# parsakhaz/multimodal-image-similarity-search

Measured on AMD Instinct MI355X. Metric: images/s CLIP-B/32 encode @ bs256; Mvec/s cosine top-10 over 10M x 512, higher is better.
Workload: dtype bf16

## Files before the change

multimodal-image-similarity-search_amd/csrc/api_index.hip:

```cpp
#include "common.h"
#include <queue>
#include "retrieval_kernels.h"
#include "gemm_bf16_256.h"
#include "gemm_bf16_p256.h"
#include <algorithm>

struct mmiss_index {
    int dim = 0, dtype = MMISS_F32, device = 0, elt = 4;
    int qelt() const { return dtype == MMISS_F32 ? 4 : 2; }
    hipStream_t own_stream = nullptr, user_stream = nullptr;
    bool has_user_stream = false;
    hipEvent_t done_ev = nullptr;
    bool async_pending = false;
    std::mutex mu;
    int64_t count = 0, capacity = 0;
    DevBuf rows, labels_d;
    DevBuf inv;
    std::vector<int64_t> labels_h;
    DevBuf tags;
    std::vector<uint64_t> tags_h;
    DevBuf fmask, fmask2, tag_stage;
    DevBuf stage, qn, qs, qstage, lists_s, lists_r, lists2_s, lists2_r, cand, cur_s, cur_r, out_c, map, gmax;
    DevBuf qmap, qmap64, qs2, cand2;
    DevBuf eps_q, thr, thr2, swp_cnt, swp_list;
    DevBuf seed_s, seed_r, fcnt, fbuf_s, fbuf_g;
    PinBuf pin;
    PinBuf swp_pin;
    int64_t stat_queries = 0, stat_flagged = 0, stat_rounds = 0, stat_pages = 0, stat_exhaustive = 0, stat_swept_rows = 0;
    struct Pending {
        bool active = false, out_dev = false, guard = false;
        int Q = 0, k = 0;
        int64_t* d_lab = nullptr; float* d_dist = nullptr; int32_t* d_cnt = nullptr; int32_t* h_flags = nullptr;
        int64_t* out_labels = nullptr; float* out_dist = nullptr; int32_t* out_count = nullptr;
        bool filt = false;
        std::vector<uint64_t> req, exc;
        const uint64_t* d_mask = nullptr;
    } pend;
    DevBuf dist_all;
    PinBuf dist_pin;
    hipStream_t stream() const { return has_user_stream ? user_stream : own_stream; }
};

#define MM_NO_PENDING(ix, who) \
    do { if ((ix)->pend.active) MM_FAIL(MMISS_ERR_STATE, "%s: a query begun with mmiss_index_query_begin is still open", who); } while (0)

namespace {

template <typename T_, typename Q_, typename Bits_> struct Storage { using T = T_; using Q = Q_; using Bits = Bits_; };
template <typename F> auto with_storage(int dtype, F&& f) {
    if (dtype == MMISS_F16) return f(Storage<_Float16, _Float16, _Float16>{});
    if (dtype == MMISS_F8) return f(Storage<F8, _Float16, uint8_t>{});
    return f(Storage<float, float, float>{});
}
template <typename S> constexpr bool is_f8 = std::is_same<typename S::T, F8>::value;

struct RowStore {
    DevBuf rows, labels, inv, tags;
    int alloc(const mmiss_index* ix, int64_t cap, hipStream_t st) {
        MM_TRY(rows.alloc((size_t)cap * ix->dim * ix->elt));
        MM_TRY(labels.alloc((size_t)cap * 8));
        MM_TRY(tags.alloc((size_t)cap * 8));
        MM_HIP(hipMemsetAsync(tags.p, 0, (size_t)cap * 8, st));
        if (ix->dtype == MMISS_F8) {
            MM_TRY(inv.alloc((size_t)cap * 4));
            MM_HIP(hipMemsetAsync(inv.p, 0, (size_t)cap * 4, st));
        }
        return MMISS_OK;
    }
};

void swap_rows(mmiss_index* ix, RowStore& s) { ix->rows.swap(s.rows); ix->labels_d.swap(s.labels); ix->inv.swap(s.inv); ix->tags.swap(s.tags); }

int reset_rows(mmiss_index* ix, hipStream_t st) {
    ix->count = 0;
    ix->labels_h.clear();
    ix->tags_h.clear();
    if (ix->capacity == 0) return MMISS_OK;
    if (ix->dtype == MMISS_F8) MM_HIP(hipMemsetAsync(ix->inv.p, 0, (size_t)ix->capacity * 4, st));
    MM_HIP(hipMemsetAsync(ix->tags.p, 0, (size_t)ix->capacity * 8, st));
    MM_HIP(hipStreamSynchronize(st));
    return MMISS_OK;
}

// ... 174 lines not shown
    if (!out) MM_FAIL(MMISS_ERR_ARG, "mmiss_index_create: null out");
    if (dim <= 0 || dim % 128 || dim > 4096) MM_FAIL(MMISS_ERR_UNSUPPORTED, "index dim %d: need a multiple of 128, <= 4096", dim);
    if (storage_dtype != MMISS_F32 && storage_dtype != MMISS_F16 && storage_dtype != MMISS_F8)
        MM_FAIL(MMISS_ERR_ARG, "unknown storage dtype %d", storage_dtype);
    if (scan_lds_bytes(dim, storage_dtype == MMISS_F32 ? 4 : 2, 1, 64) > SCAN_LDS_LIMIT)
        MM_FAIL(MMISS_ERR_UNSUPPORTED, "index dim %d with storage dtype %d: a 16-query block of the scan needs %d bytes of LDS (limit %d); "
                "f32 rows go up to dim 1920, f16 / fp8 rows up to 3968", dim, storage_dtype,
                scan_lds_bytes(dim, storage_dtype == MMISS_F32 ? 4 : 2, 1, 64), SCAN_LDS_LIMIT);
    MM_TRY(mmiss_use_device(device));
    mmiss_index* ix = new (std::nothrow) mmiss_index();
    if (!ix) MM_FAIL(MMISS_ERR_NOMEM, "out of host memory");
    ix->dim = dim; ix->dtype = storage_dtype; ix->device = device; ix->elt = storage_dtype == MMISS_F16 ? 2 : storage_dtype == MMISS_F8 ? 1 : 4;
    if (hipStreamCreateWithFlags(&ix->own_stream, hipStreamNonBlocking) != hipSuccess) {
        delete ix;
        MM_FAIL(MMISS_ERR_HIP, "hipStreamCreate failed");
    }
    if (hipEventCreateWithFlags(&ix->done_ev, hipEventDisableTiming) != hipSuccess) {
        (void)hipStreamDestroy(ix->own_stream);
        delete ix;
        MM_FAIL(MMISS_ERR_HIP, "hipEventCreate failed");
    }
    if (capacity_hint > 0) {
        int rc = index_reserve(ix, capacity_hint, ix->own_stream);
        if (rc != MMISS_OK) {
            (void)hipStreamDestroy(ix->own_stream); (void)hipEventDestroy(ix->done_ev);
            delete ix;
            return rc;
        }
    }
    *out = ix;
    return MMISS_OK;
}

extern "C" int mmiss_index_destroy(mmiss_index* ix) {
    if (!ix) return MMISS_OK;
    (void)hipSetDevice(ix->device);
    (void)hipDeviceSynchronize();
    if (ix->own_stream) (void)hipStreamDestroy(ix->own_stream);
    if (ix->done_ev) (void)hipEventDestroy(ix->done_ev);
    delete ix;
    return MMISS_OK;
}

extern "C" int mmiss_index_set_stream(mmiss_index* ix, void* hip_stream, int32_t use_own) {
    if (!ix) MM_FAIL(MMISS_ERR_ARG, "null index");
    std::lock_guard<std::mutex> lk(ix->mu);
    MM_NO_PENDING(ix, "mmiss_index_set_stream");
    hipStream_t next = reinterpret_cast<hipStream_t>(hip_stream);
    const bool next_user = use_own == 0;
    if (next_user != ix->has_user_stream || (next_user && next != ix->user_stream)) {
        MM_TRY(mmiss_use_device(ix->device));
        if (ix->async_pending) MM_HIP(hipEventSynchronize(ix->done_ev));
        ix->async_pending = false;
    }
    ix->user_stream = next;
    ix->has_user_stream = next_user;
    return MMISS_OK;
}

extern "C" int mmiss_index_count(mmiss_index* ix, int64_t* count) {
    if (!ix || !count) MM_FAIL(MMISS_ERR_ARG, "mmiss_index_count: null argument");
    std::lock_guard<std::mutex> lk(ix->mu);
    *count = ix->count;
    return MMISS_OK;
}

extern "C" int mmiss_index_clear(mmiss_index* ix) {
    if (!ix) MM_FAIL(MMISS_ERR_ARG, "null index");
    std::lock_guard<std::mutex> lk(ix->mu);
    MM_NO_PENDING(ix, "mmiss_index_clear");
    if (ix->capacity > 0) MM_TRY(mmiss_use_device(ix->device));
    return reset_rows(ix, ix->stream());
}

extern "C" int mmiss_index_add(mmiss_index* ix, const float* vecs, const int64_t* labels, int64_t n) {
    if (!ix || (n > 0 && (!vecs || !labels))) MM_FAIL(MMISS_ERR_ARG, "mmiss_index_add: null argument");
    if (n < 0) MM_FAIL(MMISS_ERR_ARG, "mmiss_index_add: n = %lld", (long long)n);
    if (n == 0) return MMISS_OK;
    std::lock_guard<std::mutex> lk(ix->mu);
    MM_NO_PENDING(ix, "mmiss_index_add");
    MM_TRY(mmiss_use_device(ix->device));
    hipStream_t st = ix->stream();
    std::vector<int64_t> lab;
    MM_TRY(fetch_i64(labels, n, lab));
    int64_t prev = ix->labels_h.empty() ? INT64_MIN : ix->labels_h.back();
    for (int64_t i = 0; i < n; ++i) {
        if (lab[i] < 0) MM_FAIL(MMISS_ERR_ARG, "mmiss_index_add: negative label %lld", (long long)lab[i]);
        if (lab[i] <= prev)
            MM_FAIL(MMISS_ERR_ARG, "mmiss_index_add: labels must be strictly increasing (label %lld after %lld)",
                    (long long)lab[i], (long long)prev);
        prev = lab[i];
    }
    if (ix->count + n >= (int64_t)INT32_MAX - 64) MM_FAIL(MMISS_ERR_UNSUPPORTED, "index shard limited to 2^31 rows");
    MM_TRY(index_reserve(ix, ix->count + n, st));
    const int D = ix->dim;
    const bool in_dev = mmiss_is_device_ptr(vecs);
    const int64_t chunk = 1 << 16;
    for (int64_t r0 = 0; r0 < n; r0 += chunk) {
        const int64_t nr = std::min(chunk, n - r0);
        const float* src = vecs + r0 * D;
        if (!in_dev) {
            MM_TRY(ix->stage.ensure((size_t)chunk * D * 4));
            MM_HIP(hipMemcpyAsync(ix->stage.p, src, (size_t)nr * D * 4, hipMemcpyHostToDevice, st));
            src = ix->stage.as<float>();
        }
        MM_TRY(launch_normalize(ix, src, ix->rows.as<char>() + (size_t)(ix->count + r0) * D * ix->elt, nr, st, ix->count + r0));
        if (!in_dev) MM_HIP(hipStreamSynchronize(st));
    }
    MM_HIP(hipMemcpyAsync(ix->labels_d.as<int64_t>() + ix->count, lab.data(), (size_t)n * 8, hipMemcpyHostToDevice, st));
    MM_HIP(hipStreamSynchronize(st));
    ix->labels_h.insert(ix->labels_h.end(), lab.begin(), lab.end());
    ix->tags_h.resize((size_t)(ix->count + n), 0);
    ix->count += n;
    return MMISS_OK;
}

extern "C" int mmiss_index_update(mmiss_index* ix, const int64_t* labels, const float* vecs, int64_t n) {
    if (!ix || (n > 0 && (!vecs || !labels))) MM_FAIL(MMISS_ERR_ARG, "mmiss_index_update: null argument");
    if (n <= 0) return n == 0 ? MMISS_OK : MMISS_ERR_ARG;
    std::lock_guard<std::mutex> lk(ix->mu);
    MM_NO_PENDING(ix, "mmiss_index_update");
    MM_TRY(mmiss_use_device(ix->device));
    hipStream_t st = ix->stream();
    std::vector<int64_t> lab;
    MM_TRY(fetch_i64(labels, n, lab));
    std::vector<int64_t> rows((size_t)n);
    for (int64_t i = 0; i < n; ++i) {
        rows[i] = find_row(ix, lab[i]);
        if (rows[i] < 0) MM_FAIL(MMISS_ERR_ARG, "mmiss_index_update: label %lld not in the index", (long long)lab[i]);
    }
    const int D = ix->dim;
    const float* src = vecs;
    if (!mmiss_is_device_ptr(vecs)) {
        MM_TRY(ix->stage.ensure((size_t)n * D * 4));
        MM_HIP(hipMemcpyAsync(ix->stage.p, vecs, (size_t)n * D * 4, hipMemcpyHostToDevice, st));
        src = ix->stage.as<float>();
    }
    for (int64_t i = 0; i < n; ++i)
        MM_TRY(launch_normalize(ix, src + i * D, ix->rows.as<char>() + (size_t)rows[i] * D * ix->elt, 1, st, rows[i]));
    MM_HIP(hipStreamSynchronize(st));
    return MMISS_OK;
}

extern "C" int mmiss_index_remove(mmiss_index* ix, const int64_t* labels, int64_t n, int64_t* removed) {
    if (!ix || (n > 0 && !labels)) MM_FAIL(MMISS_ERR_ARG, "mmiss_index_remove: null argument");
    if (removed) *removed = 0;
    if (n <= 0) return n == 0 ? MMISS_OK : MMISS_ERR_ARG;
    std::lock_guard<std::mutex> lk(ix->mu);
    MM_NO_PENDING(ix, "mmiss_index_remove");
    MM_TRY(mmiss_use_device(ix->device));
    hipStream_t st = ix->stream();
    std::vector<int64_t> lab;
    MM_TRY(fetch_i64(labels, n, lab));
    std::vector<char> drop((size_t)ix->count, 0);
    int64_t ndrop = 0;
    for (int64_t i = 0; i < n; ++i) {
        const int64_t r = find_row(ix, lab[i]);
        if (r >= 0 && !drop[r]) { drop[r] = 1; ++ndrop; }
    }
    if (removed) *removed = ndrop;
    if (ndrop == 0) return MMISS_OK;
    const int64_t keep = ix->count - ndrop;
    if (keep == 0) return reset_rows(ix, st);
    std::vector<int64_t> map((size_t)keep), nl((size_t)keep);
    std::vector<uint64_t> ntag((size_t)keep);
    for (int64_t r = 0, o = 0; r < ix->count; ++r)
        if (!drop[r]) { map[o] = r; nl[o] = ix->labels_h[r]; ntag[o] = ix->tags_h[r]; ++o; }
    RowStore fresh;
    MM_TRY(fresh.alloc(ix, ix->capacity, st));
    MM_HIP(hipMemcpyAsync(fresh.tags.p, ntag.data(), (size_t)keep * 8, hipMemcpyHostToDevice, st));
    MM_TRY(ix->map.ensure((size_t)keep * 8));
    MM_HIP(hipMemcpyAsync(ix->map.p, map.data(), (size_t)keep * 8, hipMemcpyHostToDevice, st));
    with_storage(ix->dtype, [&](auto s) {
        using B = typename decltype(s)::Bits;
        hipLaunchKernelGGL(gather_rows_kernel<B>, dim3((int)std::min<int64_t>(4096, (keep * ix->dim + 255) / 256)), dim3(256), 0, st,
                           ix->rows.as<B>(), ix->map.as<int64_t>(), fresh.rows.as<B>(), keep, ix->dim);
        if constexpr (is_f8<decltype(s)>)
            hipLaunchKernelGGL(gather_rows_kernel<float>, dim3((int)std::min<int64_t>(4096, (keep + 255) / 256)), dim3(256), 0, st,
                               ix->inv.as<float>(), ix->map.as<int64_t>(), fresh.inv.as<float>(), keep, 1);
    });
    MM_HIP(hipGetLastError());
    MM_HIP(hipMemcpyAsync(fresh.labels.p, nl.data(), (size_t)keep * 8, hipMemcpyHostToDevice, st));
    MM_HIP(hipStreamSynchronize(st));
    swap_rows(ix, fresh);
    ix->labels_h.swap(nl);
    ix->tags_h.swap(ntag);
    ix->count = keep;
    return MMISS_OK;
}

extern "C" int mmiss_index_get(mmiss_index* ix, const int64_t* labels, int64_t n, float* out) {
    if (!ix || (n > 0 && (!labels || !out))) MM_FAIL(MMISS_ERR_ARG, "mmiss_index_get: null argument");
    if (n <= 0) return n == 0 ? MMISS_OK : MMISS_ERR_ARG;
    std::lock_guard<std::mutex> lk(ix->mu);
    MM_NO_PENDING(ix, "mmiss_index_get");
    MM_TRY(mmiss_use_device(ix->device));
    hipStream_t st = ix->stream();
    std::vector<int64_t> lab;
    MM_TRY(fetch_i64(labels, n, lab));
    std::vector<int64_t> map((size_t)n);
    for (int64_t i = 0; i < n; ++i) {
        map[i] = find_row(ix, lab[i]);
// ... 146 lines not shown
            else if (Ent(d, (int32_t)r) < heap.top()) { heap.pop(); heap.push(Ent(d, (int32_t)r)); }
        }
        int32_t* c = cand.data() + (size_t)i * kkpad;
        for (size_t j = 0; !heap.empty(); ++j) { c[j] = heap.top().second; heap.pop(); }
        ix->stat_exhaustive += 1;
    }
    MM_TRY(ix->cand2.ensure((size_t)nq * kkpad * 4));
    MM_TRY(ix->qmap.ensure((size_t)nq * 4));
    MM_HIP(hipMemcpyAsync(ix->cand2.p, cand.data(), (size_t)nq * kkpad * 4, hipMemcpyHostToDevice, st));
    MM_HIP(hipMemcpyAsync(ix->qmap.p, which.data(), (size_t)nq * 4, hipMemcpyHostToDevice, st));
    RerankArgs r{};
    r.rows = ix->rows.p; r.D = D; r.inv = ix->inv.as<float>(); r.qn = ix->qn.as<float>(); r.cand = ix->cand2.as<int32_t>();
    r.cand_stride = kkpad; r.ncand = kkpad; r.group_mode = 0; r.nrows = N;
    r.labels = ix->labels_d.as<int64_t>(); r.k = pd.k;
    r.out_labels = pd.d_lab; r.out_dist = pd.d_dist; r.out_count = pd.d_cnt;
    r.qmap = ix->qmap.as<int32_t>();
    MM_TRY(launch_rerank(ix, st, r, nq));
    MM_HIP(hipStreamSynchronize(st));
    return MMISS_OK;
}

int strip_length(int Mq, int64_t nbn, int64_t ncol) {
    const int64_t tiles = nbn * (Mq / 256);
    int strip = (int)std::min<int64_t>(32, std::max<int64_t>(1, tiles / 2048));
    if (strip >= 8 && mmiss_option("score_strip_fit", 1) != 0) {
        double best = 1e300;
        int best_s = strip;
        for (int sl = strip; sl >= strip / 2; --sl) {
            const int64_t wgs = (Mq / 256) * ((ncol + sl - 1) / sl);
            const int64_t rounds = (wgs + 255) / 256;
            const double cost = (double)rounds * (sl + 0.25);
            if (cost < best - 1e-9) { best = cost; best_s = sl; }
        }
        strip = best_s;
    }
    const int forced = mmiss_option("score_strip", 0);
    if (forced > 0) strip = forced;
    return strip;
}

bool strip_v3(const mmiss_index* ix) { return mmiss_option("score_strip_v3", 1) != 0 && (ix->dim % 128) == 0 && ix->dim >= 256; }

bool strip_gemm_rows(const mmiss_index* ix) {
    return ix->dtype == MMISS_F16 || (ix->dtype == MMISS_F8 && mmiss_option("score_f8_gemm", 1) != 0);
}

int launch_strip_gemm(mmiss_index* ix, hipStream_t st, bool v3, const void* qs, const GemmEpi& ep, int M, int N, int strip,
                      const StripFilter* flt) {
    if (ix->dtype == MMISS_F8) return launch_gemm256s<_Float16, true>(st, qs, ix->rows.p, ep, M, N, ix->dim, strip, flt);
    if (v3) return launch_gemm256s<_Float16>(st, qs, ix->rows.p, ep, M, N, ix->dim, strip, flt);
    return launch_gemm256_strip<_Float16>(st, qs, ix->rows.p, ep, M, N, ix->dim, strip, flt);
}

int sweep_queries(mmiss_index* ix, hipStream_t st, const mmiss_index::Pending& pd, const std::vector<int32_t>& which) {
    const int Qf = (int)which.size(), D = ix->dim;
    const int64_t N = ix->count;
    if (Qf == 0 || N <= 0) return MMISS_OK;
    const bool gemm = !pd.filt && strip_gemm_rows(ix) && strip_v3(ix) && Qf > mmiss_option("sweep_gemm_min_q", 64);
    const int Qfp = (int)round_up(Qf, 256);
    MM_TRY(ix->swp_cnt.ensure((size_t)Qfp * 4));
    MM_TRY(ix->swp_list.ensure((size_t)Qf * SWEEP_CAP * 4));
    MM_HIP(hipMemsetAsync(ix->swp_cnt.p, 0, (size_t)Qfp * 4, st));
    const bool all = Qf == pd.Q;
    const void* qs_sw = ix->qs.p;
    const float* thr_sw = ix->thr.as<float>();
    const int32_t* qmap_sw = nullptr;
    const uint64_t* fm_sw = pd.d_mask;
    std::vector<uint64_t> fm2;
    if (!all && pd.filt) {
        fm2.resize((size_t)Qf * 2);
        for (int i = 0; i < Qf; ++i) { fm2[i] = pd.req[(size_t)which[i]]; fm2[Qf + i] = pd.exc[(size_t)which[i]]; }
        MM_TRY(ix->fmask2.ensure((size_t)Qf * 16));
        MM_HIP(hipMemcpyAsync(ix->fmask2.p, fm2.data(), (size_t)Qf * 16, hipMemcpyHostToDevice, st));
        fm_sw = ix->fmask2.as<uint64_t>();
    }
    if (!all) {
        std::vector<int64_t> map64(which.begin(), which.end());
        MM_TRY(ix->qmap.ensure((size_t)Qf * 4));
        MM_TRY(ix->qmap64.ensure((size_t)Qf * 8));
        MM_TRY(ix->qs2.ensure((size_t)Qfp * D * ix->qelt()));
        MM_TRY(ix->thr2.ensure((size_t)Qfp * 4));
        MM_HIP(hipMemcpyAsync(ix->qmap.p, which.data(), (size_t)Qf * 4, hipMemcpyHostToDevice, st));
        MM_HIP(hipMemcpyAsync(ix->qmap64.p, map64.data(), (size_t)Qf * 8, hipMemcpyHostToDevice, st));
        MM_HIP(hipStreamSynchronize(st));
        if (Qfp > Qf) MM_HIP(hipMemsetAsync(ix->qs2.as<char>() + (size_t)Qf * D * ix->qelt(), 0, (size_t)(Qfp - Qf) * D * ix->qelt(), st));
        with_storage(ix->dtype, [&](auto s) {
            using QT = typename decltype(s)::Q;
            hipLaunchKernelGGL(gather_rows_kernel<QT>, dim3((int)std::min<int64_t>(4096, ((int64_t)Qf * D + 255) / 256)), dim3(256), 0, st,
                               ix->qs.as<QT>(), ix->qmap64.as<int64_t>(), ix->qs2.as<QT>(), (int64_t)Qf, D);
        });
        MM_HIP(hipGetLastError());
        hipLaunchKernelGGL(gather_rows_kernel<float>, dim3((Qf + 255) / 256), dim3(256), 0, st, ix->thr.as<float>(),
                           ix->qmap64.as<int64_t>(), ix->thr2.as<float>(), (int64_t)Qf, 1);
        MM_HIP(hipGetLastError());
        qs_sw = ix->qs2.p; thr_sw = ix->thr2.as<float>(); qmap_sw = ix->qmap.as<int32_t>();
    }
    if (gemm) {
        const int64_t Npad = round_up(N, 256), nbn = Npad / 256;
        GemmEpi ep{};
        ep.m_valid = Qf; ep.p0 = (int)N; ep.m_fast = 1;
        ep.aux = ix->inv.as<float>();
        StripFilter flt{};
        flt.tau = thr_sw; flt.tau_stride = 1; flt.cnt = ix->swp_cnt.as<int32_t>();
        flt.buf_s = nullptr; flt.buf_g = ix->swp_list.as<int32_t>(); flt.cap = SWEEP_CAP; flt.bn_begin = 0;
        const int strip = strip_length(Qfp, nbn, nbn);
        MM_PROF(ix->dtype == MMISS_F8 ? "sweep_gemm_f8" : "sweep_gemm_f16", st, 2.0 * Qf * (double)N * D, (double)N * D * ix->elt);
        MM_TRY(launch_strip_gemm(ix, st, true, qs_sw, ep, Qfp, (int)Npad, strip, &flt));
        ix->stat_pages += 1;
    } else {
        const ScanPlan p = plan_sweep(D, ix->qelt(), Qf, N);
        if (p.lds > SCAN_LDS_LIMIT)
            MM_FAIL(MMISS_ERR_UNSUPPORTED, "widen pass: a 16-query block of dim %d does not fit the LDS (%d bytes)", D, p.lds);
        ScanArgs a{};
        a.rows = ix->rows.p; a.N = N; a.D = D; a.inv = ix->inv.as<float>(); a.qs = qs_sw; a.Q = Qf;
        a.thr = thr_sw; a.gcnt = ix->swp_cnt.as<int32_t>(); a.glist = ix->swp_list.as<int32_t>(); a.gcap = SWEEP_CAP;
        if (pd.filt) { a.tags = ix->tags.as<uint64_t>(); a.req = fm_sw; a.exc = fm_sw + Qf; }
        a.tiles_per_block = p.tiles_per_block;
        MM_TRY(launch_scan(ix, st, a, p));
        ix->stat_pages += p.qtiles;
    }
    const int SWEEP_FAST = 1024;
    RerankArgs r{};
    r.rows = ix->rows.p; r.D = D; r.inv = ix->inv.as<float>(); r.qn = ix->qn.as<float>(); r.cand = ix->swp_list.as<int32_t>();
    r.cand_stride = SWEEP_CAP; r.ncand = SWEEP_FAST; r.cand_cnt = ix->swp_cnt.as<int32_t>();
    r.group_mode = 0; r.nrows = N;
    r.labels = ix->labels_d.as<int64_t>(); r.k = pd.k;
    r.out_labels = pd.d_lab; r.out_dist = pd.d_dist; r.out_count = pd.d_cnt;
    r.qmap = qmap_sw;
    MM_TRY(ix->swp_pin.ensure((size_t)Qf * 4, st, (size_t)(Qf < 1024 ? 1024 : 2 * Qf) * 4));
    r.cnt_host = ix->swp_pin.as<int32_t>();
    MM_TRY(launch_rerank(ix, st, r, Qf));
    r.cnt_host = nullptr;
    MM_HIP(hipStreamSynchronize(st));
    const int32_t* cnt = ix->swp_pin.as<int32_t>();
    ix->stat_rounds += 1;
    std::vector<int32_t> big_b, rest;
    int maxc = 1;
    for (int b = 0; b < Qf; ++b) {
        if (cnt[b] > SWEEP_CAP) rest.push_back(which[b]);
        else {
            ix->stat_swept_rows += cnt[b];
            if (cnt[b] > SWEEP_FAST) { big_b.push_back(b); maxc = std::max(maxc, cnt[b]); }
        }
    }
    if (!big_b.empty()) {
        const int nb = (int)big_b.size();
        std::vector<int32_t> qm((size_t)nb);
        for (int j = 0; j < nb; ++j) qm[j] = which[big_b[j]];
        MM_TRY(ix->cand2.ensure((size_t)nb * 8));
        MM_HIP(hipMemcpyAsync(ix->cand2.p, big_b.data(), (size_t)nb * 4, hipMemcpyHostToDevice, st));
        MM_HIP(hipMemcpyAsync(ix->cand2.as<int32_t>() + nb, qm.data(), (size_t)nb * 4, hipMemcpyHostToDevice, st));
        MM_HIP(hipStreamSynchronize(st));
        r.ncand = (int)round_up(maxc, 32);
        r.bmap = ix->cand2.as<int32_t>();
        r.qmap = ix->cand2.as<int32_t>() + nb;
        MM_TRY(launch_rerank(ix, st, r, nb));
    }
    MM_TRY(exhaustive_queries(ix, st, pd, rest));
    MM_HIP(hipStreamSynchronize(st));
    return MMISS_OK;
}

}

namespace {

struct QueryPlan {
    int kp = 0, pages = 0, ncand = 0;
    bool dense = false;
    bool dense8 = false;
    bool big = false;
    bool strip_v3 = false;
    bool sample = false;
    int Mq = 0, strip = 1, filter_cap = 0;
    int64_t Npad = 0, nbn = 0, ns_tiles = 0, Ndense = 0;
};

int plan_query(const mmiss_index* ix, int Q, int k, bool filt, QueryPlan& p) {
    const int64_t N = ix->count;
    const int64_t want = std::min<int64_t>(k, N);
    if (want <= 10) { p.kp = 16; p.pages = 1; }
    else if (want <= 24) { p.kp = 32; p.pages = 1; }
    else {
        p.kp = 32;
        p.pages = (int)((std::min<int64_t>(want + 8, N) + 31) / 32);
    }
    p.ncand = p.kp * p.pages;
    if (p.ncand > 2048) MM_FAIL(MMISS_ERR_UNSUPPORTED, "mmiss_index_query: k = %d too large (max 2040)", k);

    const bool single = !filt && N > 0 && p.pages == 1;
    p.big = Q >= mmiss_option("score_big_min_q", 129);
    p.strip_v3 = strip_v3(ix);
    p.dense8 = single && ix->dtype == MMISS_F8 && p.big && p.strip_v3 && strip_gemm_rows(ix);
    p.dense = (single && ix->dtype == MMISS_F16 && Q > 16) || p.dense8;
    if (!p.dense) return MMISS_OK;
    p.Npad = round_up(N, p.big ? 256 : 128);
    p.Mq = (int)round_up(Q, p.big ? 256 : 128);
    p.nbn = p.Npad / 256;
    p.ns_tiles = std::max<int64_t>(16, p.nbn / std::max(1, mmiss_option("score_sample_div", 32)));
    const int filter_opt = mmiss_option("score_filter", 1);
    p.sample = p.big && p.nbn >= 128 && filter_opt != 0 && (filter_opt == 2 || (double)p.Mq * (double)p.Npad >= 1e9);
    p.Ndense = p.sample ? p.ns_tiles * 256 : p.Npad;
    if (p.big) p.strip = strip_length(p.Mq, p.nbn, p.sample ? p.nbn - p.ns_tiles : p.nbn);
    if (p.sample) p.filter_cap = mmiss_option("score_filter_cap", 2048);
    return MMISS_OK;
}

int stage_filter(mmiss_index* ix, hipStream_t st, int Q, const uint64_t* req, const uint64_t* exc) {
    mmiss_index::Pending& pd = ix->pend;
    pd.filt = req || exc;
    pd.d_mask = nullptr;
    if (!pd.filt) return MMISS_OK;
    if (req) MM_TRY(fetch_u64(req, Q, pd.req, st)); else pd.req.assign((size_t)Q, 0);
// ... 129 lines not shown
        MM_HIP(hipMemcpyAsync(ix->cur_s.p, inf.data(), (size_t)Q * 4, hipMemcpyHostToDevice, st));
        MM_HIP(hipMemcpyAsync(ix->cur_r.p, neg.data(), (size_t)Q * 4, hipMemcpyHostToDevice, st));
        MM_HIP(hipStreamSynchronize(st));
    }
    for (int page = 0; page < qp.pages; ++page) {
        ScanArgs a{};
        a.rows = ix->rows.p; a.N = ix->count; a.D = ix->dim; a.inv = ix->inv.as<float>(); a.qs = ix->qs.p; a.Q = Q;
        a.cur_s = paging ? ix->cur_s.as<float>() : nullptr;
        a.cur_r = paging ? ix->cur_r.as<int32_t>() : nullptr;
        a.kp = kp; a.tiles_per_block = p.tiles_per_block;
        a.out_s = ix->lists_s.as<float>(); a.out_r = ix->lists_r.as<int32_t>();
        if (pd.filt) { a.tags = ix->tags.as<uint64_t>(); a.req = pd.d_mask; a.exc = pd.d_mask + Q; }
        MM_TRY(launch_scan(ix, st, a, p));
        MergeArgs m{};
        m.in_s = ix->lists_s.as<float>(); m.in_r = ix->lists_r.as<int32_t>();
        m.L = p.slabs; m.Q = Q; m.kp = kp;
        m.cand = ix->cand.as<int32_t>(); m.cand_stride = qp.ncand; m.page_off = page * kp;
        m.cur_s = ix->cur_s.as<float>(); m.cur_r = ix->cur_r.as<int32_t>();
        MM_TRY(launch_merge(ix, st, m));
    }
    return MMISS_OK;
}

int rerank_first(mmiss_index* ix, hipStream_t st, const QueryPlan& p) {
    const mmiss_index::Pending& pd = ix->pend;
    RerankArgs r{};
    r.rows = ix->rows.p; r.D = ix->dim; r.inv = ix->inv.as<float>(); r.qn = ix->qn.as<float>(); r.cand = ix->cand.as<int32_t>();
    r.cand_stride = p.ncand; r.ncand = p.dense ? p.ncand * 16 : p.ncand; r.group_mode = p.dense ? 1 : 0; r.nrows = ix->count;
    r.labels = ix->labels_d.as<int64_t>(); r.k = pd.k;
    r.out_labels = pd.d_lab; r.out_dist = pd.d_dist; r.out_count = pd.d_cnt;
    if (pd.guard) {
        r.tau = ix->cur_s.as<float>(); r.eps_q = ix->eps_q.as<float>();
        r.thr_out = ix->thr.as<float>();
        r.flags = pd.h_flags; r.nflag = nullptr;
        r.force_flag = mmiss_option("guard_force", 0);
        if (p.sample) { r.ovf_cnt = ix->fcnt.as<int32_t>(); r.ovf_cap = p.filter_cap; }
    }
    return launch_rerank(ix, st, r, pd.Q);
}

int query_begin_locked(mmiss_index* ix, const float* queries, int32_t Q, int32_t k, const uint64_t* req, const uint64_t* exc,
                       int64_t* out_labels, float* out_dist, int32_t* out_count) {
    MM_TRY(mmiss_use_device(ix->device));
    hipStream_t st = ix->stream();
    const int64_t N = ix->count;
    mmiss_index::Pending& pd = ix->pend;
    pd.out_dev = mmiss_is_device_ptr(out_labels);
    if (pd.out_dev != mmiss_is_device_ptr(out_dist) || (out_count && pd.out_dev != mmiss_is_device_ptr(out_count)))
        MM_FAIL(MMISS_ERR_ARG, "mmiss_index_query: output pointers must be all host or all device");
    MM_TRY(stage_filter(ix, st, Q, req, exc));
    MM_TRY(stage_outputs(ix, st, Q, k, out_labels, out_dist, out_count));
    QueryPlan p;
    MM_TRY(plan_query(ix, Q, k, pd.filt, p));
    MM_TRY(upload_queries(ix, st, queries, Q));
    MM_TRY(ix->cand.ensure((size_t)Q * p.ncand * 4));
    MM_TRY(ix->cur_s.ensure((size_t)Q * 4));
    MM_TRY(ix->cur_r.ensure((size_t)Q * 4));
    if (N == 0) MM_HIP(hipMemsetAsync(ix->cand.p, 0xff, (size_t)Q * p.ncand * 4, st));
    else if (p.dense) MM_TRY(dense_pass(ix, st, p, Q));
    else MM_TRY(scan_pass(ix, st, p, Q));
    pd.guard = N > 0 && mmiss_option("exact_guard", 1) != 0;
    MM_TRY(rerank_first(ix, st, p));
    ix->stat_queries += Q;
    MM_HIP(hipEventRecord(ix->done_ev, st));
    pd.active = true;
    return MMISS_OK;
}

int query_end_locked(mmiss_index* ix) {
    const mmiss_index::Pending& pd = ix->pend;
    ix->pend.active = false;
    MM_TRY(mmiss_use_device(ix->device));
    hipStream_t st = ix->stream();
    if (!pd.guard && pd.out_dev && ix->has_user_stream) {
        ix->async_pending = true;
        return MMISS_OK;
    }
    MM_HIP(hipEventSynchronize(ix->done_ev));
    if (pd.guard) {
        std::vector<int32_t> which;
        for (int q = 0; q < pd.Q; ++q)
            if (pd.h_flags[q]) which.push_back(q);
        if (!which.empty()) {
            ix->stat_flagged += (int64_t)which.size();
            MM_TRY(sweep_queries(ix, st, pd, which));
        }
    }
    if (!pd.out_dev) {
        memcpy(pd.out_labels, pd.d_lab, (size_t)pd.Q * pd.k * 8);
        memcpy(pd.out_dist, pd.d_dist, (size_t)pd.Q * pd.k * 4);
        if (pd.out_count) memcpy(pd.out_count, pd.d_cnt, (size_t)pd.Q * 4);
    }
    return MMISS_OK;
}

int query_entry(mmiss_index* ix, const float* queries, int32_t Q, int32_t k, const uint64_t* req, const uint64_t* exc,
                int64_t* out_labels, float* out_dist, int32_t* out_count, bool begin_only, const char* who) {
    if (!ix || !queries || !out_labels || !out_dist) MM_FAIL(MMISS_ERR_ARG, "%s: null argument", who);
    if (Q < 0 || k <= 0) MM_FAIL(MMISS_ERR_ARG, "%s: Q=%d k=%d", who, Q, k);
    if (Q == 0) {
        if (begin_only) MM_FAIL(MMISS_ERR_ARG, "%s: Q = 0", who);
        return MMISS_OK;
    }
    std::lock_guard<std::mutex> lk(ix->mu);
    MM_NO_PENDING(ix, who);
    MM_TRY(query_begin_locked(ix, queries, Q, k, req, exc, out_labels, out_dist, out_count));
    return begin_only ? MMISS_OK : query_end_locked(ix);
}

}

extern "C" int mmiss_index_query(mmiss_index* ix, const float* queries, int32_t Q, int32_t k, int64_t* out_labels,
                                 float* out_dist, int32_t* out_count) {
    return query_entry(ix, queries, Q, k, nullptr, nullptr, out_labels, out_dist, out_count, false, "mmiss_index_query");
}

extern "C" int mmiss_index_query_begin(mmiss_index* ix, const float* queries, int32_t Q, int32_t k, int64_t* out_labels,
                                       float* out_dist, int32_t* out_count) {
    return query_entry(ix, queries, Q, k, nullptr, nullptr, out_labels, out_dist, out_count, true, "mmiss_index_query_begin");
}

extern "C" int mmiss_index_query_filtered(mmiss_index* ix, const float* queries, int32_t Q, int32_t k, const uint64_t* require,
                                          const uint64_t* exclude, int64_t* out_labels, float* out_dist, int32_t* out_count) {
    return query_entry(ix, queries, Q, k, require, exclude, out_labels, out_dist, out_count, false, "mmiss_index_query_filtered");
}

extern "C" int mmiss_index_query_filtered_begin(mmiss_index* ix, const float* queries, int32_t Q, int32_t k, const uint64_t* require,
                                                const uint64_t* exclude, int64_t* out_labels, float* out_dist, int32_t* out_count) {
    return query_entry(ix, queries, Q, k, require, exclude, out_labels, out_dist, out_count, true, "mmiss_index_query_filtered_begin");
}

extern "C" int mmiss_index_query_end(mmiss_index* ix) {
    if (!ix) MM_FAIL(MMISS_ERR_ARG, "mmiss_index_query_end: null index");
    std::lock_guard<std::mutex> lk(ix->mu);
    if (!ix->pend.active) MM_FAIL(MMISS_ERR_STATE, "mmiss_index_query_end: no query was begun");
    return query_end_locked(ix);
}

extern "C" int mmiss_index_query_abort(mmiss_index* ix) {
    if (!ix) MM_FAIL(MMISS_ERR_ARG, "mmiss_index_query_abort: null index");
    std::lock_guard<std::mutex> lk(ix->mu);
    if (!ix->pend.active) return MMISS_OK;
    ix->pend.active = false;
    MM_TRY(mmiss_use_device(ix->device));
    MM_HIP(hipEventSynchronize(ix->done_ev));
    return MMISS_OK;
}

extern "C" int mmiss_index_guard_stats_ex(mmiss_index* ix, int64_t out[8]) {
    if (!ix || !out) MM_FAIL(MMISS_ERR_ARG, "mmiss_index_guard_stats_ex: null argument");
    std::lock_guard<std::mutex> lk(ix->mu);
    for (int i = 0; i < 8; ++i) out[i] = 0;
    out[0] = ix->stat_queries; out[1] = ix->stat_flagged; out[2] = ix->stat_rounds; out[3] = ix->stat_pages;
    out[4] = ix->stat_exhaustive; out[5] = ix->stat_swept_rows;
    return MMISS_OK;
}

extern "C" int mmiss_index_guard_stats(mmiss_index* ix, int64_t out[4]) {
    if (!ix || !out) MM_FAIL(MMISS_ERR_ARG, "mmiss_index_guard_stats: null argument");
    std::lock_guard<std::mutex> lk(ix->mu);
    out[0] = ix->stat_queries; out[1] = ix->stat_flagged; out[2] = ix->stat_rounds; out[3] = ix->stat_pages;
    return MMISS_OK;
}

namespace {
struct IdxHeader {
    char magic[8];
    int32_t version, dim, dtype, reserved;
    int64_t count;
};

int load_rows(mmiss_index* ix, FILE* f, const char* path, int64_t n, const std::vector<int64_t>& lab, hipStream_t st) {
    const size_t row_bytes = (size_t)ix->dim * ix->elt;
    const int64_t chunk = std::max<int64_t>(1, (64 << 20) / (int64_t)row_bytes);
    std::vector<char> buf((size_t)std::min<int64_t>(chunk, std::max<int64_t>(n, 1)) * row_bytes);
    for (int64_t r0 = 0; r0 < n; r0 += chunk) {
        const int64_t nr = std::min(chunk, n - r0);
        if (fread(buf.data(), row_bytes, (size_t)nr, f) != (size_t)nr ||
            hipMemcpy(ix->rows.as<char>() + (size_t)r0 * row_bytes, buf.data(), (size_t)nr * row_bytes, hipMemcpyHostToDevice) != hipSuccess)
            MM_FAIL(MMISS_ERR_IO, "%s could not be read to its end", path);
    }
    if (n) MM_HIP(hipMemcpy(ix->labels_d.p, lab.data(), (size_t)n * 8, hipMemcpyHostToDevice));
    if (ix->dtype == MMISS_F8 && ix->capacity > 0) {
        MM_HIP(hipMemsetAsync(ix->inv.p, 0, (size_t)ix->capacity * 4, st));
        MM_TRY(launch_f8_inv(ix, 0, n, st));
        MM_HIP(hipStreamSynchronize(st));
    }
    if (ix->capacity > 0) {
        MM_HIP(hipMemsetAsync(ix->tags.p, 0, (size_t)ix->capacity * 8, st));
        MM_HIP(hipStreamSynchronize(st));
    }
    return MMISS_OK;
}
}

extern "C" int mmiss_index_save(mmiss_index* ix, const char* path) {
    if (!ix || !path) MM_FAIL(MMISS_ERR_ARG, "mmiss_index_save: null argument");
    std::lock_guard<std::mutex> lk(ix->mu);
    MM_NO_PENDING(ix, "mmiss_index_save");
    MM_TRY(mmiss_use_device(ix->device));
    MM_HIP(hipStreamSynchronize(ix->stream()));
    FILE* f = fopen(path, "wb");
    if (!f) MM_FAIL(MMISS_ERR_IO, "cannot open %s for writing", path);
    IdxHeader h{};
    memcpy(h.magic, "MMISSIDX", 8);
    h.version = 1; h.dim = ix->dim; h.dtype = ix->dtype; h.count = ix->count;
    bool ok = fwrite(&h, sizeof(h), 1, f) == 1;
    if (ok && ix->count) ok = fwrite(ix->labels_h.data(), 8, (size_t)ix->count, f) == (size_t)ix->count;
    const size_t row_bytes = (size_t)ix->dim * ix->elt;
    const int64_t chunk = std::max<int64_t>(1, (64 << 20) / (int64_t)row_bytes);
    std::vector<char> buf((size_t)std::min<int64_t>(chunk, std::max<int64_t>(ix->count, 1)) * row_bytes);
    for (int64_t r0 = 0; ok && r0 < ix->count; r0 += chunk) {
        const int64_t nr = std::min(chunk, ix->count - r0);
        if (hipMemcpy(buf.data(), ix->rows.as<char>() + (size_t)r0 * row_bytes, (size_t)nr * row_bytes,
                      hipMemcpyDeviceToHost) != hipSuccess) { ok = false; break; }
        ok = fwrite(buf.data(), row_bytes, (size_t)nr, f) == (size_t)nr;
    }
    ok = (fclose(f) == 0) && ok;
    if (!ok) MM_FAIL(MMISS_ERR_IO, "write to %s failed", path);
    return MMISS_OK;
}

extern "C" int mmiss_index_load(mmiss_index* ix, const char* path) {
    if (!ix || !path) MM_FAIL(MMISS_ERR_ARG, "mmiss_index_load: null argument");
    std::lock_guard<std::mutex> lk(ix->mu);
    MM_NO_PENDING(ix, "mmiss_index_load");
    MM_TRY(mmiss_use_device(ix->device));
    hipStream_t st = ix->stream();
    FILE* f = fopen(path, "rb");
    if (!f) MM_FAIL(MMISS_ERR_IO, "cannot open %s", path);
    IdxHeader h{};
    if (fread(&h, sizeof(h), 1, f) != 1 || memcmp(h.magic, "MMISSIDX", 8) != 0 || h.version != 1) {
        fclose(f);
        MM_FAIL(MMISS_ERR_IO, "%s is not an mmiss index file", path);
    }
    if (h.dim != ix->dim || h.dtype != ix->dtype || h.count < 0) {
        fclose(f);
        MM_FAIL(MMISS_ERR_ARG, "%s holds dim %d dtype %d; this index is dim %d dtype %d", path, h.dim, h.dtype, ix->dim,
                ix->dtype);
    }
    const size_t row_bytes = (size_t)ix->dim * ix->elt;
    {
        const long at = ftell(f);
        long end = -1;
        if (at >= 0 && fseek(f, 0, SEEK_END) == 0) end = ftell(f);
        if (at < 0 || end < 0 || fseek(f, at, SEEK_SET) != 0) { fclose(f); MM_FAIL(MMISS_ERR_IO, "cannot seek in %s", path); }
        if ((uint64_t)h.count > (uint64_t)(end - at) / (8 + row_bytes)) {
            fclose(f);
            MM_FAIL(MMISS_ERR_IO, "%s is truncated or corrupt (%ld bytes behind the header, %lld rows need %llu); the index is unchanged",
                    path, end - at, (long long)h.count, (unsigned long long)((uint64_t)h.count * (8 + row_bytes)));
        }
    }
    std::vector<int64_t> lab((size_t)h.count);
    bool ok = h.count == 0 || fread(lab.data(), 8, (size_t)h.count, f) == (size_t)h.count;
    for (int64_t i = 1; ok && i < h.count; ++i) ok = lab[i] > lab[i - 1];
    if (!ok) { fclose(f); MM_FAIL(MMISS_ERR_IO, "%s: labels unreadable or not strictly increasing; the index is unchanged", path); }
    int rc = index_reserve(ix, h.count, st);
    if (rc != MMISS_OK) { fclose(f); return rc; }
    rc = load_rows(ix, f, path, h.count, lab, st);
    fclose(f);
    if (rc != MMISS_OK) {
        const std::string why = mmiss_last_error();
        (void)reset_rows(ix, st);
        MM_FAIL(rc, "%s; the index was cleared", why.c_str());
    }
    ix->tags_h.assign((size_t)h.count, 0);
    ix->labels_h.swap(lab);
    ix->count = h.count;
    return MMISS_OK;
}

extern "C" int mmiss_blend(int device, void* hip_stream, const float* img, const float* txt, double w, int32_t Q,
                           int32_t dim, float* out) {
    if (!img || !txt || !out) MM_FAIL(MMISS_ERR_ARG, "mmiss_blend: null argument");
    if (Q < 0 || dim <= 0 || dim % 64) MM_FAIL(MMISS_ERR_ARG, "mmiss_blend: Q=%d dim=%d (dim must be a multiple of 64)", Q, dim);
    if (Q == 0) return MMISS_OK;
    MM_TRY(mmiss_use_device(device));
    hipStream_t st = reinterpret_cast<hipStream_t>(hip_stream);
    const size_t bytes = (size_t)Q * dim * 4;
// ... 73 lines not shown
```

multimodal-image-similarity-search_amd/index.py:

```python
from __future__ import annotations

import ctypes as C
import threading
from typing import Optional, Tuple

import numpy as np

from . import _lib

F32, F16, F8 = _lib.MMISS_F32, _lib.MMISS_F16, _lib.MMISS_F8
_DTYPES = {"f32": F32, "float32": F32, "f16": F16, "float16": F16, "f8": F8, "fp8": F8, "e4m3": F8, F32: F32, F16: F16, F8: F8}


def _is_torch(x) -> bool:
    return hasattr(x, "data_ptr")


class FlatIndex:
    def __init__(self, dim: int, dtype="f32", device: int = 0, capacity: int = 0):
        self.dim = int(dim)
        self.dtype = _DTYPES[dtype]
        self.device = int(device)
        self._lib = _lib.load()
        h = C.c_void_p()
# ... 137 lines not shown
                _lib.check(self._lib.mmiss_index_query_begin(self._h, _lib.ptr(q), int(q.shape[0]), int(k), _lib.ptr(outs[0]), _lib.ptr(outs[1]),
                                                             _lib.ptr(outs[2])))
            else:
                _lib.check(self._lib.mmiss_index_query_filtered_begin(self._h, _lib.ptr(q), int(q.shape[0]), int(k), _lib.ptr(masks[0]),
                                                                      _lib.ptr(masks[1]), _lib.ptr(outs[0]), _lib.ptr(outs[1]), _lib.ptr(outs[2])))
            self._query_gen += 1
            return prev, PendingQuery(self, q, outs, self._query_gen, masks)

    def _masks(self, q, require, exclude):
        if require is None and exclude is None:
            return None
        Q = int(q.shape[0])
        return (self._mask(require, Q, q, "require"), self._mask(exclude, Q, q, "exclude"))

    def _prepare(self, queries, k: int):
        q = self._vecs(queries)
        Q = int(q.shape[0])
        if _is_torch(q) and q.is_cuda:
            import torch

            lab = torch.empty((Q, k), dtype=torch.int64, device=q.device)
            dist = torch.empty((Q, k), dtype=torch.float32, device=q.device)
            cnt = torch.empty((Q,), dtype=torch.int32, device=q.device)
        else:
            if _is_torch(q):
                q = q.numpy()
            lab = np.empty((Q, k), dtype=np.int64)
            dist = np.empty((Q, k), dtype=np.float32)
            cnt = np.empty((Q,), dtype=np.int32)
        return q, (lab, dist, cnt)

    def _query(self, queries, k: int, split: bool, require=None, exclude=None):
        q, (lab, dist, cnt) = self._prepare(queries, k)
        Q = int(q.shape[0])
        masks = self._masks(q, require, exclude)
        with self._call_lock:
            self._sync_stream(q)
            if masks is None:
                fn = self._lib.mmiss_index_query_begin if split else self._lib.mmiss_index_query
                _lib.check(fn(self._h, _lib.ptr(q), Q, int(k), _lib.ptr(lab), _lib.ptr(dist), _lib.ptr(cnt)))
            else:
                fn = self._lib.mmiss_index_query_filtered_begin if split else self._lib.mmiss_index_query_filtered
                _lib.check(fn(self._h, _lib.ptr(q), Q, int(k), _lib.ptr(masks[0]), _lib.ptr(masks[1]), _lib.ptr(lab), _lib.ptr(dist),
                              _lib.ptr(cnt)))
            if split:
                self._query_gen += 1
                return PendingQuery(self, q, (lab, dist, cnt), self._query_gen, masks)
        return (lab, dist, cnt)

    def guard_stats(self) -> dict:
        out = (C.c_int64 * 8)()
        _lib.check(self._lib.mmiss_index_guard_stats_ex(self._h, out))
        return {"queries": out[0], "widened": out[1], "rounds": out[2], "pages": out[3], "exhaustive": out[4],
                "swept_rows": out[5]}

    def save(self, path: str) -> None:
        _lib.check(self._lib.mmiss_index_save(self._h, str(path).encode()))

    def load(self, path: str) -> None:
        _lib.check(self._lib.mmiss_index_load(self._h, str(path).encode()))

    def abort_query(self) -> None:
        with self._call_lock:
            self._query_gen += 1
            _lib.check(self._lib.mmiss_index_query_abort(self._h))

    def close(self):
        if getattr(self, "_h", None):
            with self._call_lock:
                self._query_gen += 1
                self._lib.mmiss_index_query_abort(self._h)
                self._lib.mmiss_index_destroy(self._h)
                self._h = None

    def __del__(self):
        try:
            self.close()
        except Exception:
            pass


class PendingQuery:

    def __init__(self, index: "FlatIndex", q, outs, gen: int, masks=None):
        self._index, self._q, self._outs, self._gen, self._done = index, q, outs, gen, False
        self._masks = masks

    def _current(self) -> bool:
        idx = self._index
        return getattr(idx, "_h", None) is not None and idx._query_gen == self._gen

    def result(self):
        if not self._done:
            idx = self._index
            with idx._call_lock:
                if not self._current():
                    self._done = True
                    self._q = None
                    raise RuntimeError("this query was aborted (FlatIndex.abort_query / close, or a later query_begin)")
                self._done = True
                idx._query_gen += 1
                _lib.check(idx._lib.mmiss_index_query_end(idx._h))
            self._q = None
        return self._outs

    def abort(self) -> None:
        if not self._done:
# ... 69 lines not shown
```

Baseline: 87800.

## Speculatively queue exact-guard sweep with the first query pass when most queries get flagged

Adds an adaptive speculative mode. When the exact guard has flagged at least 90% of queries on two consecutive calls, the full GEMM sweep for every query is queued at query-begin time, right behind the first rerank. This removes the host round trip (sync, read flags, then launch the sweep) that would otherwise serialize the widening pass. The cost is extra sweep work for queries that would not have been flagged, so mode is left once the flagged share drops below 50%. It also refactors the sweep into queue and finish steps and adds a speculative statistic.

```diff
diff --git a/multimodal-image-similarity-search_amd/csrc/api_index.hip b/multimodal-image-similarity-search_amd/csrc/api_index.hip
--- a/multimodal-image-similarity-search_amd/csrc/api_index.hip
+++ b/multimodal-image-similarity-search_amd/csrc/api_index.hip
@@ -27,8 +27,14 @@
     PinBuf pin;
     PinBuf swp_pin;
     int64_t stat_queries = 0, stat_flagged = 0, stat_rounds = 0, stat_pages = 0, stat_exhaustive = 0, stat_swept_rows = 0;
+    int64_t stat_speculative = 0;
+    int spec_streak = 0;
+    bool spec_on = false;
+    void spec_reset() { spec_streak = 0; spec_on = false; }
     struct Pending {
         bool active = false, out_dev = false, guard = false;
+        bool spec_eligible = false;
+        bool spec = false;
         int Q = 0, k = 0;
         int64_t* d_lab = nullptr; float* d_dist = nullptr; int32_t* d_cnt = nullptr; int32_t* h_flags = nullptr;
         int64_t* out_labels = nullptr; float* out_dist = nullptr; int32_t* out_count = nullptr;
@@ -309,6 +315,7 @@
         MM_TRY(mmiss_use_device(ix->device));
         if (ix->async_pending) MM_HIP(hipEventSynchronize(ix->done_ev));
         ix->async_pending = false;
+        ix->spec_reset();
     }
     ix->user_stream = next;
     ix->has_user_stream = next_user;
@@ -326,6 +333,7 @@
     if (!ix) MM_FAIL(MMISS_ERR_ARG, "null index");
     std::lock_guard<std::mutex> lk(ix->mu);
     MM_NO_PENDING(ix, "mmiss_index_clear");
+    ix->spec_reset();
     if (ix->capacity > 0) MM_TRY(mmiss_use_device(ix->device));
     return reset_rows(ix, ix->stream());
 }
@@ -336,6 +344,7 @@
     if (n == 0) return MMISS_OK;
     std::lock_guard<std::mutex> lk(ix->mu);
     MM_NO_PENDING(ix, "mmiss_index_add");
+    ix->spec_reset();
     MM_TRY(mmiss_use_device(ix->device));
     hipStream_t st = ix->stream();
     std::vector<int64_t> lab;
@@ -377,6 +386,7 @@
     if (n <= 0) return n == 0 ? MMISS_OK : MMISS_ERR_ARG;
     std::lock_guard<std::mutex> lk(ix->mu);
     MM_NO_PENDING(ix, "mmiss_index_update");
+    ix->spec_reset();
     MM_TRY(mmiss_use_device(ix->device));
     hipStream_t st = ix->stream();
     std::vector<int64_t> lab;
@@ -405,6 +415,7 @@
     if (n <= 0) return n == 0 ? MMISS_OK : MMISS_ERR_ARG;
     std::lock_guard<std::mutex> lk(ix->mu);
     MM_NO_PENDING(ix, "mmiss_index_remove");
+    ix->spec_reset();
     MM_TRY(mmiss_use_device(ix->device));
     hipStream_t st = ix->stream();
     std::vector<int64_t> lab;
@@ -657,16 +668,39 @@
     return launch_gemm256_strip<_Float16>(st, qs, ix->rows.p, ep, M, N, ix->dim, strip, flt);
 }
 
-int sweep_queries(mmiss_index* ix, hipStream_t st, const mmiss_index::Pending& pd, const std::vector<int32_t>& which) {
-    const int Qf = (int)which.size(), D = ix->dim;
+constexpr int SWEEP_FAST = 1024;
+
+bool sweep_on_gemm(const mmiss_index* ix, bool filt, int Qf) {
+    return !filt && strip_gemm_rows(ix) && strip_v3(ix) && Qf > mmiss_option("sweep_gemm_min_q", 64);
+}
+
+int sweep_reserve(mmiss_index* ix, hipStream_t st, int Qf) {
+    MM_TRY(ix->swp_cnt.ensure((size_t)round_up(Qf, 256) * 4));
+    MM_TRY(ix->swp_list.ensure((size_t)Qf * SWEEP_CAP * 4));
+    MM_TRY(ix->swp_pin.ensure((size_t)Qf * 4, st, (size_t)(Qf < 1024 ? 1024 : 2 * Qf) * 4));
+    return MMISS_OK;
+}
+
+RerankArgs sweep_rerank_args(const mmiss_index* ix, const mmiss_index::Pending& pd, const int32_t* qmap) {
+    RerankArgs r{};
+    r.rows = ix->rows.p; r.D = ix->dim; r.inv = ix->inv.as<float>(); r.qn = ix->qn.as<float>(); r.cand = ix->swp_list.as<int32_t>();
+    r.cand_stride = SWEEP_CAP; r.ncand = SWEEP_FAST; r.cand_cnt = ix->swp_cnt.as<int32_t>();
+    r.group_mode = 0; r.nrows = ix->count;
+    r.labels = ix->labels_d.as<int64_t>(); r.k = pd.k;
+    r.out_labels = pd.d_lab; r.out_dist = pd.d_dist; r.out_count = pd.d_cnt;
+    r.qmap = qmap;
+    return r;
+}
+
+int sweep_queue(mmiss_index* ix, hipStream_t st, const mmiss_index::Pending& pd, const int32_t* which, int Qf) {
+    const int D = ix->dim;
     const int64_t N = ix->count;
     if (Qf == 0 || N <= 0) return MMISS_OK;
-    const bool gemm = !pd.filt && strip_gemm_rows(ix) && strip_v3(ix) && Qf > mmiss_option("sweep_gemm_min_q", 64);
+    const bool gemm = sweep_on_gemm(ix, pd.filt, Qf);
     const int Qfp = (int)round_up(Qf, 256);
-    MM_TRY(ix->swp_cnt.ensure((size_t)Qfp * 4));
-    MM_TRY(ix->swp_list.ensure((size_t)Qf * SWEEP_CAP * 4));
+    MM_TRY(sweep_reserve(ix, st, Qf));
     MM_HIP(hipMemsetAsync(ix->swp_cnt.p, 0, (size_t)Qfp * 4, st));
-    const bool all = Qf == pd.Q;
+    const bool all = which == nullptr;
     const void* qs_sw = ix->qs.p;
     const float* thr_sw = ix->thr.as<float>();
     const int32_t* qmap_sw = nullptr;
@@ -680,12 +714,12 @@
         fm_sw = ix->fmask2.as<uint64_t>();
     }
     if (!all) {
-        std::vector<int64_t> map64(which.begin(), which.end());
+        std::vector<int64_t> map64(which, which + Qf);
         MM_TRY(ix->qmap.ensure((size_t)Qf * 4));
         MM_TRY(ix->qmap64.ensure((size_t)Qf * 8));
         MM_TRY(ix->qs2.ensure((size_t)Qfp * D * ix->qelt()));
         MM_TRY(ix->thr2.ensure((size_t)Qfp * 4));
-        MM_HIP(hipMemcpyAsync(ix->qmap.p, which.data(), (size_t)Qf * 4, hipMemcpyHostToDevice, st));
+        MM_HIP(hipMemcpyAsync(ix->qmap.p, which, (size_t)Qf * 4, hipMemcpyHostToDevice, st));
         MM_HIP(hipMemcpyAsync(ix->qmap64.p, map64.data(), (size_t)Qf * 8, hipMemcpyHostToDevice, st));
         MM_HIP(hipStreamSynchronize(st));
         if (Qfp > Qf) MM_HIP(hipMemsetAsync(ix->qs2.as<char>() + (size_t)Qf * D * ix->qelt(), 0, (size_t)(Qfp - Qf) * D * ix->qelt(), st));
@@ -724,19 +758,15 @@
         MM_TRY(launch_scan(ix, st, a, p));
         ix->stat_pages += p.qtiles;
     }
-    const int SWEEP_FAST = 1024;
-    RerankArgs r{};
-    r.rows = ix->rows.p; r.D = D; r.inv = ix->inv.as<float>(); r.qn = ix->qn.as<float>(); r.cand = ix->swp_list.as<int32_t>();
-    r.cand_stride = SWEEP_CAP; r.ncand = SWEEP_FAST; r.cand_cnt = ix->swp_cnt.as<int32_t>();
-    r.group_mode = 0; r.nrows = N;
-    r.labels = ix->labels_d.as<int64_t>(); r.k = pd.k;
-    r.out_labels = pd.d_lab; r.out_dist = pd.d_dist; r.out_count = pd.d_cnt;
-    r.qmap = qmap_sw;
-    MM_TRY(ix->swp_pin.ensure((size_t)Qf * 4, st, (size_t)(Qf < 1024 ? 1024 : 2 * Qf) * 4));
+    RerankArgs r = sweep_rerank_args(ix, pd, qmap_sw);
     r.cnt_host = ix->swp_pin.as<int32_t>();
-    MM_TRY(launch_rerank(ix, st, r, Qf));
-    r.cnt_host = nullptr;
-    MM_HIP(hipStreamSynchronize(st));
+    return launch_rerank(ix, st, r, Qf);
+}
+
+int sweep_finish(mmiss_index* ix, hipStream_t st, const mmiss_index::Pending& pd, const std::vector<int32_t>& which,
+                 const int32_t* counted) {
+    const int Qf = (int)which.size();
+    if (Qf == 0 || ix->count <= 0) return MMISS_OK;
     const int32_t* cnt = ix->swp_pin.as<int32_t>();
     ix->stat_rounds += 1;
     std::vector<int32_t> big_b, rest;
@@ -744,11 +774,12 @@
     for (int b = 0; b < Qf; ++b) {
         if (cnt[b] > SWEEP_CAP) rest.push_back(which[b]);
         else {
-            ix->stat_swept_rows += cnt[b];
+            if (!counted || counted[which[b]]) ix->stat_swept_rows += cnt[b];
             if (cnt[b] > SWEEP_FAST) { big_b.push_back(b); maxc = std::max(maxc, cnt[b]); }
         }
     }
     if (!big_b.empty()) {
+        RerankArgs r = sweep_rerank_args(ix, pd, nullptr);
         const int nb = (int)big_b.size();
         std::vector<int32_t> qm((size_t)nb);
         for (int j = 0; j < nb; ++j) qm[j] = which[big_b[j]];
@@ -762,8 +793,30 @@
         MM_TRY(launch_rerank(ix, st, r, nb));
     }
     MM_TRY(exhaustive_queries(ix, st, pd, rest));
+    if (!big_b.empty()) MM_HIP(hipStreamSynchronize(st));
+    return MMISS_OK;
+}
+
+int sweep_queries(mmiss_index* ix, hipStream_t st, const mmiss_index::Pending& pd, const std::vector<int32_t>& which) {
+    const int Qf = (int)which.size();
+    if (Qf == 0 || ix->count <= 0) return MMISS_OK;
+    MM_TRY(sweep_queue(ix, st, pd, Qf == pd.Q ? nullptr : which.data(), Qf));
     MM_HIP(hipStreamSynchronize(st));
-    return MMISS_OK;
+    return sweep_finish(ix, st, pd, which, nullptr);
+}
+
+constexpr int SPEC_ENTER_CALLS = 2;
+constexpr int SPEC_ENTER_PCT = 90;
+constexpr int SPEC_LEAVE_PCT = 50;
+
+void spec_record(mmiss_index* ix, int nflag, int Q) {
+    if (ix->spec_on) {
+        if ((int64_t)nflag * 100 < (int64_t)SPEC_LEAVE_PCT * Q) ix->spec_reset();
+    } else if ((int64_t)nflag * 100 >= (int64_t)SPEC_ENTER_PCT * Q) {
+        if (++ix->spec_streak >= SPEC_ENTER_CALLS) ix->spec_on = true;
+    } else {
+        ix->spec_streak = 0;
+    }
 }
 
 }
@@ -999,6 +1052,11 @@
     MM_TRY(stage_outputs(ix, st, Q, k, out_labels, out_dist, out_count));
     QueryPlan p;
     MM_TRY(plan_query(ix, Q, k, pd.filt, p));
+    pd.guard = N > 0 && mmiss_option("exact_guard", 1) != 0;
+    pd.spec_eligible = pd.guard && mmiss_option("guard_force", 0) == 0 && p.dense && !p.sample && sweep_on_gemm(ix, pd.filt, Q);
+    const int spec_opt = mmiss_option("speculative_widen", 1);
+    pd.spec = pd.spec_eligible && (spec_opt == 2 || (spec_opt == 1 && ix->spec_on));
+    if (pd.spec) MM_TRY(sweep_reserve(ix, st, Q));
     MM_TRY(upload_queries(ix, st, queries, Q));
     MM_TRY(ix->cand.ensure((size_t)Q * p.ncand * 4));
     MM_TRY(ix->cur_s.ensure((size_t)Q * 4));
@@ -1006,9 +1064,12 @@
     if (N == 0) MM_HIP(hipMemsetAsync(ix->cand.p, 0xff, (size_t)Q * p.ncand * 4, st));
     else if (p.dense) MM_TRY(dense_pass(ix, st, p, Q));
     else MM_TRY(scan_pass(ix, st, p, Q));
-    pd.guard = N > 0 && mmiss_option("exact_guard", 1) != 0;
     MM_TRY(rerank_first(ix, st, p));
     ix->stat_queries += Q;
+    if (pd.spec) {
+        MM_TRY(sweep_queue(ix, st, pd, nullptr, Q));
+        ix->stat_speculative += 1;
+    }
     MM_HIP(hipEventRecord(ix->done_ev, st));
     pd.active = true;
     return MMISS_OK;
@@ -1028,8 +1089,14 @@
         std::vector<int32_t> which;
         for (int q = 0; q < pd.Q; ++q)
             if (pd.h_flags[q]) which.push_back(q);
-        if (!which.empty()) {
-            ix->stat_flagged += (int64_t)which.size();
+        const int nflag = (int)which.size();
+        ix->stat_flagged += nflag;
+        if (pd.spec_eligible) spec_record(ix, nflag, pd.Q);
+        if (pd.spec) {
+            which.resize((size_t)pd.Q);
+            for (int q = 0; q < pd.Q; ++q) which[(size_t)q] = q;
+            MM_TRY(sweep_finish(ix, st, pd, which, pd.h_flags));
+        } else if (nflag > 0) {
             MM_TRY(sweep_queries(ix, st, pd, which));
         }
     }
@@ -1099,7 +1166,7 @@
     std::lock_guard<std::mutex> lk(ix->mu);
     for (int i = 0; i < 8; ++i) out[i] = 0;
     out[0] = ix->stat_queries; out[1] = ix->stat_flagged; out[2] = ix->stat_rounds; out[3] = ix->stat_pages;
-    out[4] = ix->stat_exhaustive; out[5] = ix->stat_swept_rows;
+    out[4] = ix->stat_exhaustive; out[5] = ix->stat_swept_rows; out[6] = ix->stat_speculative;
     return MMISS_OK;
 }
 
@@ -1172,6 +1239,7 @@
     if (!ix || !path) MM_FAIL(MMISS_ERR_ARG, "mmiss_index_load: null argument");
     std::lock_guard<std::mutex> lk(ix->mu);
     MM_NO_PENDING(ix, "mmiss_index_load");
+    ix->spec_reset();
     MM_TRY(mmiss_use_device(ix->device));
     hipStream_t st = ix->stream();
     FILE* f = fopen(path, "rb");
diff --git a/multimodal-image-similarity-search_amd/index.py b/multimodal-image-similarity-search_amd/index.py
--- a/multimodal-image-similarity-search_amd/index.py
+++ b/multimodal-image-similarity-search_amd/index.py
@@ -213,7 +213,7 @@
         out = (C.c_int64 * 8)()
         _lib.check(self._lib.mmiss_index_guard_stats_ex(self._h, out))
         return {"queries": out[0], "widened": out[1], "rounds": out[2], "pages": out[3], "exhaustive": out[4],
-                "swept_rows": out[5]}
+                "swept_rows": out[5], "speculative": out[6]}
 
     def save(self, path: str) -> None:
         _lib.check(self._lib.mmiss_index_save(self._h, str(path).encode()))
```

After: 88700 (median of 6 runs). 1.01x the previous value.
